# grantjr1842/delayed-streams-modeling

Measured on AMD Instinct MI355X. Metric: real-time stream throughput, stt-1b-en_fr @ bs=64 per GPU (Mimi encode + LM decode per 80 ms frame), higher is better.
Workload: dtype bf16 weights + bf16 KV, f32 activations as three exact bf16 pieces, f32 accumulate (v_mfma_f32_16x16x32_bf16); 1 GPU; stt-1b-en_fr batch=64 streaming, ring KV cache full (750 frames), Mimi encode + LM decode HIP path; streams_per_gpu=64, parallelism=replicas x1 (independent stream batches, no per-step collective), streams=encoder stream || 2 LM group stream(s)

## Files before the change

delayed-streams-modeling_amd/csrc/dsm_engine.hip:

```cpp
#include <hip/hip_runtime.h>

#include <cmath>
#include <cstdarg>
#include <cstdio>
#include <cstdlib>
#include <cstring>
#include <atomic>
#include <mutex>
#include <shared_mutex>
#include <string>
#include <set>
#include <vector>

#include "../../include/dsm.h"
#include "dsm_device.h"
#include "dsm_config_presets.h"
#include "dsm_kernels.h"
#include "dsm_numerics.h"
#include "dsm_safetensors.h"

static thread_local std::string g_create_error;

static int dsm_env_int(const char* name, int dflt) {
  const char* v = getenv(name);
// ... 163 lines not shown
};

struct LmState {
  ActScratch act;
  float *hidden = nullptr, *logits = nullptr, *eh = nullptr, *prs = nullptr;
  uint32_t *next_cb = nullptr, *text_token = nullptr, *text_out = nullptr, *codes_in = nullptr;
  uint8_t *first_step = nullptr, *mask = nullptr;
  uint32_t* rng_key = nullptr;
  unsigned long long* rng_pos = nullptr;
  uint8_t* gmask = nullptr;
  TransformerState tr;
  struct Group {
    int b0 = 0, nb = 0;
    TransformerState view;
  };
  std::vector<Group> groups;
};

struct HostItem {
  size_t step_idx = 0;
  std::vector<uint32_t> word_tokens;
  bool unended_word = false;
  double last_stop_time = 0.0;
};

}

struct dsm_engine : DsmDevice {
  dsm_asr_config cfg{};
  int B = 0;
  hipEvent_t ev_grp_in[kMaxGroups] = {}, ev_stagger[kMaxGroups] = {};
  bool grp_busy = false;
  bool serialize_groups = false;
  hipEvent_t ev_codes_consumed = nullptr;
  bool codes_consumed_valid = false;
  hipEvent_t ev_join = nullptr, ev_a = nullptr, ev_b = nullptr, ev_c = nullptr, ev_d = nullptr;
  MimiW mimi_w;
  MimiState mimi[2];
  std::atomic<bool> mimi1_ready{false};
  std::mutex mimi1_mu;
  MimiDecState dec;
  LmW lm_w;
  LmState lm;
  GraphSlot *g_enc[2] = {}, *g_grp[kMaxGroups] = {};
  float* h_pcm = nullptr;
  float* h_pcm1 = nullptr;
  uint8_t* h_mask = nullptr;
  uint32_t *h_codes = nullptr, *h_text = nullptr;
  float* h_prs = nullptr;
  std::vector<HostItem> items;
  size_t model_step_idx = 0;
  std::vector<dsm_asr_msg> msgs;
  std::vector<uint32_t> msg_tokens;
  dsm_metrics metrics{};
  static constexpr int kPipe = 4;
  struct PipeSlot {
    float* h_pcm = nullptr;
    uint8_t* h_mask = nullptr;
    uint32_t* d_codes = nullptr;
    hipEvent_t ev_done = nullptr, ev_consumed = nullptr;
    bool in_flight = false;
  };
  PipeSlot pipe[kPipe];
  int pipe_next = 0;
  bool pipe_ready = false;
  std::mutex pipe_mu;
};
// ... 520 lines not shown
template <typename WT, typename KVT, int EPI, int NT>
int launch_gemm_tiled(DsmDevice* e, hipStream_t st, GemmArgs& a) {
  int chunks = (a.Kpad + DSM_KC - 1) / DSM_KC;
  const int gx = (a.N + 63) / 64;
  const bool bx3 = e->dot_mode == 1 && sizeof(WT) == 2;
  auto ok4 = [](const RowMap& m) { return m.ld % 4 == 0 && m.bstride % 4 == 0; };
  a.vec = (a.N % 4 == 0) && (!a.Y || ok4(a.ymap)) && (!a.Y2 || ok4(a.y2map)) && (!a.res || ok4(a.rmap));
  a.chunk_loop = 0;
  if (chunks > 1 && (long)gx * ((a.M + 63) / 64) >= e->chunk_loop_min_tiles) {
    a.chunk_loop = chunks;
    a.defer_reduce = 0;
    chunks = 1;
  }
  if constexpr (EPI == EPI_GATE && NT == 2) {
    if (wk_applicable(e, sizeof(WT) == 2, a.Kpad, a.K, a.M) && chunks > 1 && a.N % 16 == 0) {
      a.ts = e->timeline ? e->dev_ts_slot(e->tag_gemm[e->sid(st)], e->sid(st), 1, 2) : nullptr;
      const int ph = e->prof_begin(e->tag_gemm[e->sid(st)], st);
      hipLaunchKernelGGL((gemm_wk_kernel<KVT, 1, 2, EPI_GATE, 1, 4, 2, true, 4>), dim3(a.N / 16, 1, (a.M + 15) / 16), dim3(256),
                         (size_t)chunks * 2 * 1024, st, a);
      e->prof_end(ph, st);
      HIPCHK(hipGetLastError());
      return 0;
    }
  }
  int MT = a.M > 32 ? 4 : (a.M > 16 ? 2 : 1);
  while (MT > 1 && (long)gx * chunks * ((a.M + 16 * MT - 1) / (16 * MT)) < 256) MT /= 2;
  if (MT == 4 && bx3 && chunks > 1 && a.M <= 64 && (long)gx * chunks <= 256 && EPI == EPI_STORE) MT = 2;
  const bool smallk = chunks == 1 && a.chunk_loop == 0 && (long)gx * ((a.M + 63) / 64) >= e->smallk_min_tiles && !bx3;
  if (smallk && e->smallk_mt < MT) MT = e->smallk_mt;
  a.ws_ntiles = (((NT - 1) * a.nt_stride) >> 4) + gx * 4;
  const int mtiles = (a.M + 15) / 16;
  if (chunks > 1) {
    const int wsid = e->sid(st);
    size_t need = (size_t)chunks * mtiles * a.ws_ntiles * 256 * sizeof(float);
    if (need > e->gemm_ws_cap[wsid]) {
      if (e->capturing) {
        e->capture_failed = true;
        e->set_error("split-K workspace grew during a graph capture");
        return DSM_ERR_STATE;
      }
      e->ws_gen += 1;
      HIPCHK(hipStreamSynchronize(st));
      if (e->gemm_ws[wsid]) HIPCHK(hipFree(e->gemm_ws[wsid]));
      e->gemm_ws[wsid] = nullptr;
      e->gemm_ws_cap[wsid] = 0;
      void* p = nullptr;
      HIPCHK(hipMalloc(&p, need));
      e->gemm_ws[wsid] = reinterpret_cast<float*>(p);
      e->gemm_ws_cap[wsid] = need;
    }
    a.ws = e->gemm_ws[wsid];
  }
  dim3 grid(gx, chunks, (a.M + 16 * MT - 1) / (16 * MT));
  const bool nt2 = NT == 1 && bx3 && a.chunk_loop > 1 && MT == 4 && (EPI == EPI_STORE || EPI == EPI_QKV) && a.N % 128 == 0 &&
                   (long)(a.N / 128) * grid.z >= 256;
  if (nt2) {
    grid.x = a.N / 128;
    a.wg_cols = 128;
    a.nt_stride = 64;
  }
  a.ts = e->timeline ? e->dev_ts_slot(e->tag_gemm[e->sid(st)], e->sid(st), 1, 2) : nullptr;
  const int ph = e->prof_begin(e->tag_gemm[e->sid(st)], st);
  const bool roll = a.chunk_loop > 1 || smallk;
  const bool deep = LoopDepth<WT, NT>::MAX == 4 && e->loop_depth == 4 && !smallk;
  if (nt2) hipLaunchKernelGGL((gemm_bx3_kernel<KVT, 4, (NT == 1 ? 2 : NT), (EPI == EPI_GATE ? EPI_STORE : EPI), true>), grid, dim3(256), 0, st, a);
  else if (MT == 4) launch_tile<WT, KVT, EPI, NT, 4>(st, grid, a, bx3, roll, deep);
  else if (MT == 2) launch_tile<WT, KVT, EPI, NT, 2>(st, grid, a, bx3, roll, deep);
  else launch_tile<WT, KVT, EPI, NT, 1>(st, grid, a, bx3, roll, deep);
  const bool rows_ok = (EPI == EPI_STORE) && a.norm_out && a.vec && !a.Y2 && a.Y && a.N <= 4096 && a.ymap.bstride == 0;
  if (chunks > 1 && !((EPI == EPI_QKV || EPI == EPI_STORE) && a.defer_reduce)) {
    if (rows_ok) {
      if (a.N <= 1024) hipLaunchKernelGGL(gemm_reduce_rows_kernel<1>, dim3(a.M), dim3(256), 0, st, a, chunks);
      else if (a.N <= 2048) hipLaunchKernelGGL(gemm_reduce_rows_kernel<2>, dim3(a.M), dim3(512), 0, st, a, chunks);
      else hipLaunchKernelGGL(gemm_reduce_rows_kernel<4>, dim3(a.M), dim3(1024), 0, st, a, chunks);
    } else {
      const int out_tiles = mtiles * ((a.N + 15) / 16);
      hipLaunchKernelGGL((gemm_reduce_kernel<KVT, EPI>), dim3((out_tiles + 3) / 4), dim3(256), 0, st, a, chunks);
    }
  }
  e->prof_end(ph, st);
  HIPCHK(hipGetLastError());
  if (a.norm_out && !(chunks > 1 && rows_ok)) {
    hipLaunchKernelGGL(row_norm_kernel, dim3(a.M), dim3(256), 0, st, a.norm_out, a.Y, a.norm_w, a.norm_b, a.M,
                       a.N, a.norm_eps, a.norm_rms);
// ... 171 lines not shown
```

delayed-streams-modeling_amd/csrc/dsm_engine_api.inc:

```

namespace {

template <typename KVT, int HD, int T>
int launch_attn_t(DsmDevice* e, hipStream_t st, float* out, const float* q, const void* k, const void* v,
                  const uint32_t* start_pos, const uint8_t* active, int B, int H, int ctx, int d, const AttnFused& fq) {
  constexpr int UNR = (sizeof(KVT) == 2 && T == 1 && HD == 128) ? 8 : 4;
  size_t lds = sizeof(float) * ((size_t)T * ctx + 4 * T * HD + 16);
  if ((long)B * H >= 2048 && (size_t)2 * ctx * HD * sizeof(KVT) >= (size_t)256 * 1024) lds += e->attn_lds_pad;
  if (lds > 64 * 1024) {
    static size_t allowed = 0;
    if (lds > allowed) {
      HIPCHK(hipFuncSetAttribute(reinterpret_cast<const void*>(&attn_kernel<KVT, HD, T, UNR>), hipFuncAttributeMaxDynamicSharedMemorySize, (int)lds));
      allowed = lds;
    }
  }
  const int tag = e->tag_attn[e->sid(st)];
  if (T == 1 && HD == 64 && ctx <= 32) {
    const int ph = e->prof_begin(tag, st);
    hipLaunchKernelGGL((attn_small_kernel<KVT, 64>), dim3((B * H + 3) / 4), dim3(256), 0, st, out, q, reinterpret_cast<const KVT*>(k),
                       reinterpret_cast<const KVT*>(v), start_pos, active, B * H, H, ctx, d, fq);
    e->prof_end(ph, st);
    HIPCHK(hipGetLastError());
    return 0;
  }
// ... 360 lines not shown
      const int per_b = T_out * (sw.out_c / 4);
      hipLaunchKernelGGL(convtr_overlap_add_kernel, dim3((per_b + 255) / 256 < 64 ? (per_b + 255) / 256 : 64, B), dim3(256), 0,
                         st, o);
      HIPCHK(hipGetLastError());
    }
    if (int rc = run_conv(e, st, sw.ra, ss.cat_ra, B, nullptr, none, ss.cat_rb, cat_map(sw.rb), nullptr, none)) return rc;
    if (i + 1 < w.dec_stages.size()) {
      if (int rc = run_conv(e, st, sw.rb, ss.cat_rb, B, nullptr, none, s.stages[i + 1].x, plain_map(B * T_out, sw.out_c), ss.y,
                            plain_map(B * T_out, sw.out_c)))
        return rc;
    } else {
      if (int rc = run_conv(e, st, sw.rb, ss.cat_rb, B, nullptr, none, s.cat_final, cat_map(w.dec_final), ss.y,
                            plain_map(B * T_out, sw.out_c)))
        return rc;
    }
  }
  if (int rc = run_conv(e, st, w.dec_final, s.cat_final, B, s.pcm, plain_map(B * DSM_FRAME_SIZE, c.channels), nullptr, none,
                        nullptr, none))
    return rc;
  if (!s.h_descs.empty()) {
    hipLaunchKernelGGL(conv_state_shift_kernel, dim3(B, (unsigned)s.h_descs.size()), dim3(256), 0, st, s.descs, s.mask,
                       s.first_call ? 1 : 0, s.started);
    HIPCHK(hipGetLastError());
  }
  s.first_call = false;
  return 0;
}

int lm_group_body(dsm_engine* e, hipStream_t st, int g, uint32_t* d_text_out, float* d_prs_out, int phase) {
  const dsm_asr_config& c = e->cfg;
  LmState& s = e->lm;
  const LmW& w = e->lm_w;
  LmState::Group& grp = s.groups[g];
  const int B = e->B, d = c.lm.d_model, b0 = grp.b0, nb = grp.nb;
  e->tag_gemm[e->sid(st)] = DSM_PROF_GEMM_LM;
  e->tag_attn[e->sid(st)] = DSM_PROF_ATTN_LM;
  uint8_t* gmask = s.gmask + b0;
  const ActScratch sc = s.act.from_row(b0, d, w.tr.hidden);
  float* hidden = s.hidden + (size_t)b0 * d;
  int rc = with_kv_type(c.kv_bf16 != 0, [&](auto kv) {
    return transformer_forward<uint16_t, decltype(kv)>(e, st, w.tr, grp.view, sc, nb, 1, gmask, nullptr, plain_map(1, 1), w.out_norm, hidden, phase);
  });
  if (rc || phase == 1) return rc;
  float* logits = s.logits + (size_t)b0 * c.text_out_vocab_size;
  {
    GemmArgs a = base_args(w.text_linear, hidden, plain_map(nb, d), nb);
    a.Y = logits; a.ymap = plain_map(nb, c.text_out_vocab_size);
    if ((rc = gemm_store<uint16_t>(e, st, a))) return rc;
  }
  if (c.temperature > 0.0f)
    hipLaunchKernelGGL(lm_gumbel_kernel, dim3(nb), dim3(256), 0, st, logits, c.text_out_vocab_size, c.temperature,
                       s.rng_key + (size_t)b0 * 8, s.rng_pos + b0, d_text_out + b0, s.text_token + b0, s.first_step + b0, gmask);
  else
    hipLaunchKernelGGL(lm_argmax_kernel, dim3(nb), dim3(256), 0, st, logits, c.text_out_vocab_size, d_text_out + b0,
                       s.text_token + b0, s.first_step + b0, gmask);
  HIPCHK(hipGetLastError());
  if (c.extra_heads_num > 0 && d_prs_out) {
    const int ehw = c.extra_heads_num * c.extra_heads_dim;
    float* eh = s.eh + (size_t)b0 * ehw;
    GemmArgs a = base_args(w.extra_heads, hidden, plain_map(nb, d), nb);
    a.Y = eh; a.ymap = plain_map(nb, ehw);
    if ((rc = gemm_store<uint16_t>(e, st, a))) return rc;
    int n = nb * c.extra_heads_num;
    hipLaunchKernelGGL(extra_heads_kernel, dim3((n + 255) / 256), dim3(256), 0, st, eh, d_prs_out + b0, nb,
                       c.extra_heads_num, c.extra_heads_dim, B);
    HIPCHK(hipGetLastError());
  }
  return 0;
}

int lm_group_head(dsm_engine* e, hipStream_t st, int g, const uint32_t* d_codes, const uint8_t* d_mask, bool with_prefix) {
  const dsm_asr_config& c = e->cfg;
  LmState& s = e->lm;
  const LmW& w = e->lm_w;
  LmState::Group& grp = s.groups[g];
  const int d = c.lm.d_model, b0 = grp.b0, nb = grp.nb, nc = c.audio_codebooks;
  uint8_t* gmask = s.gmask + b0;
  HIPCHK(hipMemcpyAsync(gmask, d_mask + b0, (size_t)nb, hipMemcpyDeviceToDevice, st));
  float* x = s.act.x + (size_t)b0 * d;
  hipLaunchKernelGGL(lm_input_kernel, dim3(nb, (d + 511) / 512), dim3(256), 0, st, x, w.text_emb, w.audio_emb,
                     d_codes + (size_t)b0 * nc, s.next_cb + (size_t)b0 * nc, s.text_token + b0, s.first_step + b0, gmask, nc, d,
                     c.audio_vocab_size, (uint32_t)c.audio_vocab_size - 1, (uint32_t)c.text_in_vocab_size - 1);
  hipLaunchKernelGGL(lm_next_codebooks_kernel, dim3((nb * nc + 255) / 256), dim3(256), 0, st, d_codes + (size_t)b0 * nc,
                     s.next_cb + (size_t)b0 * nc, gmask, nb, nc);
  HIPCHK(hipGetLastError());
  if (g > 0) HIPCHK(hipEventRecord(e->ev_grp_in[g], st));
  if (with_prefix)
    if (int rc = lm_group_body(e, st, g, nullptr, nullptr, 1)) return rc;
  return 0;
}

int lm_group_rest(dsm_engine* e, hipStream_t st, int g, uint32_t* d_text_out, float* d_prs_out, bool after_prefix) {
  const uint64_t key = (uint64_t)e->sid(st) ^ ((uint64_t)(uintptr_t)d_text_out << 3) ^ ((uint64_t)(uintptr_t)d_prs_out * 0x9E3779B97F4A7C15ull) ^
                       (after_prefix ? 0x8000000000000000ull : 0ull);
  return run_captured(e, *e->g_grp[g], st, key, [&] { return lm_group_body(e, st, g, d_text_out, d_prs_out, after_prefix ? 2 : 0); });
}

int wait_group_inputs(dsm_engine* e) {
  if (!e->grp_busy) return 0;
  for (size_t g = 1; g < e->lm.groups.size(); ++g) HIPCHK(hipStreamWaitEvent(e->s_model, e->ev_grp_in[g], 0));
  return 0;
}
int join_groups(dsm_engine* e) { return e->grp_busy ? join_groups(e, e->s_model, e->lm.groups.size()) : 0; }

int lm_step(dsm_engine* e, hipStream_t st, const uint32_t* d_codes, const uint8_t* d_mask, uint32_t* d_text_out,
            float* d_prs_out) {
  const size_t G = e->lm.groups.size();
  if (int rc = fork_groups(e, st, G)) return rc;
  const bool stagger = G > 1 && !e->serialize_groups && e->lm.groups[0].nb >= 256;
  for (size_t g = 0; g < G; ++g) {
    hipStream_t gs = (g == 0 || e->serialize_groups) ? st : e->s_grp[g];
    if (stagger && g > 0) HIPCHK(hipStreamWaitEvent(gs, e->ev_stagger[g - 1], 0));
    if (int rc = lm_group_head(e, gs, (int)g, d_codes, d_mask, stagger)) return rc;
    if (stagger && g + 1 < G) HIPCHK(hipEventRecord(e->ev_stagger[g], gs));
  }
  if (int rc = run_groups(e, st, G, e->serialize_groups,
                          [&](size_t g, hipStream_t gs) { return lm_group_rest(e, gs, (int)g, d_text_out, d_prs_out, stagger); }))
    return rc;
  if (G > 1) e->grp_busy = true;
// ... 177 lines not shown
  if (c.extra_heads_num > 0) {
    std::vector<float> eh((size_t)c.extra_heads_num * c.extra_heads_dim * d);
    for (int i = 0; i < c.extra_heads_num && !ld.failed; ++i) {
      auto w = ld.get((int64_t)c.extra_heads_dim * d, "extra_heads.%d.weight", i);
      memcpy(&eh[(size_t)i * c.extra_heads_dim * d], w.data(), sizeof(float) * w.size());
    }
    if (ld.failed) return DSM_ERR_IO;
    if (int rc = pack_linear(e, &e->lm_w.extra_heads, eh.data(), c.extra_heads_num * c.extra_heads_dim, d, true, nullptr)) return rc;
  }
  return 0;
}

static int create_impl(dsm_engine* e, const dsm_asr_config* cfg, int device_id, int batch_size, const char* lm_path,
                       const char* mimi_path, const void* attach_arena = nullptr, size_t attach_bytes = 0,
                       const uint8_t* attach_manifest = nullptr, size_t attach_manifest_bytes = 0) {
  e->cfg = *cfg;
  e->B = batch_size;
  const dsm_asr_config& c = e->cfg;
  if (batch_size <= 0) { e->set_error("batch_size must be positive"); return DSM_ERR_INVALID; }
  if (c.audio_codebooks > 64 || c.audio_codebooks != c.mimi.quantizer_n_q) {
    e->set_error("audio_codebooks (%d) must equal the Mimi quantizer_n_q (%d) and be <= 64", c.audio_codebooks,
                 c.mimi.quantizer_n_q);
    return DSM_ERR_INVALID;
  }
  if (c.mimi.n_residual_layers != 1) {
    e->set_error("only n_residual_layers = 1 (dilation 1 residual blocks, Mimi v0_1) is supported");
    return DSM_ERR_INVALID;
  }
  if (c.extra_heads_num > DSM_MAX_EXTRA_HEADS) { e->set_error("too many extra heads"); return DSM_ERR_INVALID; }
  if (c.dot_mode != 0 && c.dot_mode != 1) { e->set_error("dot_mode must be 0 (f32 MFMA chain) or 1 (bx3)"); return DSM_ERR_INVALID; }
  for (const dsm_transformer_config* t : {&c.lm, &c.mimi.transformer})
    if (int rc = check_transformer_config(e, *t)) return rc;
  if (int rc = e->open(device_id, c.dot_mode, true)) return rc;
  for (hipEvent_t* ev : {&e->ev_join, &e->ev_codes_consumed})
    if (int rc = e->new_event(ev)) return rc;
  for (hipEvent_t* ev : {&e->ev_a, &e->ev_b, &e->ev_c, &e->ev_d})
    if (int rc = e->new_event(ev, hipEventDefault)) return rc;
  for (auto& gs : e->g_enc) gs = e->graph_slot();
  const int B = batch_size, d = c.lm.d_model;
  if (attach_arena) {
    e->arena = const_cast<char*>(reinterpret_cast<const char*>(attach_arena));
    e->arena_size = attach_bytes;
    e->arena_owned = false;
    e->manifest.assign(attach_manifest, attach_manifest + attach_manifest_bytes);
    e->manifest_pos = 0;
    e->arena_off = 0;
    e->wmode = dsm_engine::W_ATTACH;
    if (int rc = load_all_weights(e, nullptr, nullptr)) return rc;
    if (e->arena_off != e->arena_size || e->manifest_pos != e->manifest.size()) {
      e->set_error("received weight arena does not match this configuration (%zu of %zu bytes, %zu of %zu manifest entries used)",
                   e->arena_off, e->arena_size, e->manifest_pos, e->manifest.size());
      return DSM_ERR_INVALID;
    }
  } else {
    char err[512];
    dsm_st_file* fm = dsm_st_open(mimi_path, err, sizeof err);
    if (!fm) { e->set_error("%s", err); return DSM_ERR_IO; }
    dsm_st_file* fl = dsm_st_open(lm_path, err, sizeof err);
    if (!fl) { dsm_st_close(fm); e->set_error("%s", err); return DSM_ERR_IO; }
    e->wmode = dsm_engine::W_MEASURE;
    e->arena_off = 0;
    int rc = load_all_weights(e, fl, fm);
    if (rc == 0) {
      e->arena_size = e->arena_off;
      void* p = nullptr;
      hipError_t he = hipMalloc(&p, e->arena_size);
      if (he != hipSuccess) { e->set_error("hipMalloc of the %zu-byte weight arena failed: %s", e->arena_size, hipGetErrorString(he)); rc = DSM_ERR_DEVICE; }
      else {
// ... 27 lines not shown
  if (int rc = e->dalloc(&s.next_cb, (size_t)B * c.audio_codebooks)) return rc;
  if (int rc = e->dalloc(&s.text_token, B)) return rc;
  if (int rc = e->dalloc(&s.text_out, B)) return rc;
  if (int rc = e->dalloc(&s.codes_in, (size_t)B * c.audio_codebooks)) return rc;
  if (int rc = e->dalloc(&s.first_step, B)) return rc;
  if (int rc = e->dalloc(&s.rng_key, (size_t)B * 8)) return rc;
  if (int rc = e->dalloc(&s.rng_pos, B)) return rc;
  {
    std::vector<uint32_t> keys((size_t)B * 8);
    for (int b = 0; b < B; ++b) dsm_seed_from_u64(0x5EED0000ull + (uint64_t)b, &keys[(size_t)b * 8]);
    HIPCHK(hipMemcpy(s.rng_key, keys.data(), sizeof(uint32_t) * keys.size(), hipMemcpyHostToDevice));
    HIPCHK(hipStreamSynchronize(nullptr));
  }
  if (int rc = e->dalloc(&s.mask, B)) return rc;
  if (int rc = alloc_transformer_state(e, &s.tr, c.lm, B, 1, c.kv_bf16 != 0)) return rc;
  if (int rc = e->dalloc(&s.gmask, B)) return rc;
  {
    int G = dsm_env_int("DSM_LM_GROUPS", B >= 32 ? 2 : 1);
    if (G < 1) G = 1;
    if (G > dsm_engine::kMaxGroups) G = dsm_engine::kMaxGroups;
    const int n16 = (B + 15) / 16;
    if (G > n16) G = n16;
    s.groups.resize(G);
    int b0 = 0;
    for (int g = 0; g < G; ++g) {
      int blocks = n16 / G + (g < n16 % G ? 1 : 0);
      int nb = std::min(blocks * 16, B - b0);
      LmState::Group& grp = s.groups[g];
      grp.b0 = b0;
      grp.nb = nb;
      grp.view = group_view(s.tr, c.lm, c.kv_bf16 ? 2 : 4, b0);
      b0 += nb;
      e->g_grp[g] = e->graph_slot();
      if (g > 0)
        if (int rc = e->new_event(&e->ev_grp_in[g])) return rc;
    }
    if (int rc = e->open_groups(G)) return rc;
    for (int g = 0; g + 1 < G; ++g)
      if (int rc = e->new_event(&e->ev_stagger[g])) return rc;
  }
  {
    long n = (long)B * c.audio_codebooks;
    hipLaunchKernelGGL(fill_u32_kernel, dim3((unsigned)((n + 255) / 256)), dim3(256), 0, e->s_model, s.next_cb,
                       (uint32_t)c.audio_vocab_size - 1, n);
    hipLaunchKernelGGL(fill_u32_kernel, dim3((unsigned)((B + 255) / 256)), dim3(256), 0, e->s_model, s.text_token,
                       (uint32_t)c.text_in_vocab_size - 1, (long)B);
    HIPCHK(hipGetLastError());
    HIPCHK(hipMemsetAsync(s.first_step, 1, B, e->s_model));
  }
  e->items.assign(B, HostItem());
  if (int rc = e->halloc(&e->h_pcm, (size_t)B * DSM_FRAME_SIZE)) return rc;
  if (int rc = e->halloc(&e->h_pcm1, (size_t)B * DSM_FRAME_SIZE)) return rc;
  if (int rc = e->halloc(&e->h_mask, (size_t)B)) return rc;
  if (int rc = e->halloc(&e->h_codes, (size_t)B * c.audio_codebooks)) return rc;
  if (int rc = e->halloc(&e->h_text, (size_t)B)) return rc;
  if (int rc = e->halloc(&e->h_prs, (size_t)B * (c.extra_heads_num + 1))) return rc;
  HIPCHK(hipDeviceSynchronize());
  e->metrics.algorithmic_bytes_lm = lm_algorithmic_bytes(e);
  e->metrics.algorithmic_bytes_encode = mimi_enc_algorithmic_bytes(e);
  return 0;
}

int dsm_asr_create(const dsm_asr_config* cfg, int device_id, int batch_size, const char* lm_safetensors,
                   const char* mimi_safetensors, dsm_engine** out) {
  if (!cfg || !out || !lm_safetensors || !mimi_safetensors) {
    g_create_error = "null argument";
    return DSM_ERR_INVALID;
  }
// ... 341 lines not shown
  HIPCHK(hipSetDevice(e->device));
  ApiShared api(e);
  if (int rc = dsm_sync(e)) return rc;
  uint32_t key[8];
  dsm_seed_from_u64(seed, key);
  const unsigned long long zero = 0;
  HIPCHK(hipMemcpy(e->lm.rng_key + (size_t)slot * 8, key, sizeof key, hipMemcpyHostToDevice));
  HIPCHK(hipMemcpy(e->lm.rng_pos + slot, &zero, sizeof zero, hipMemcpyHostToDevice));
  return dsm_sync(e);
}

int dsm_mimi_reset_slot(dsm_engine* e, int slot) {
  if (!e) return DSM_ERR_INVALID;
  if (slot < 0 || slot >= e->B) {
    e->set_error("batch index out of range: %d >= %d", slot, e->B);
    return DSM_ERR_INVALID;
  }
  HIPCHK(hipSetDevice(e->device));
  ApiShared api(e);
  return reset_mimi_slot(e, 0, e->s_enc, slot);
}

int dsm_get_metrics(dsm_engine* e, dsm_metrics* out) {
  if (!e || !out) return DSM_ERR_INVALID;
  *out = e->metrics;
  e->fill_graph_metrics(out);
  return 0;
}

int dsm_mimi_encode_step_dev(dsm_engine* e, const float* d_pcm, const uint8_t* d_mask, uint32_t* d_codes_out) {
  if (!e || !d_pcm || !d_mask) return DSM_ERR_INVALID;
  HIPCHK(hipSetDevice(e->device));
  ApiShared api(e);
  if (e->codes_consumed_valid) HIPCHK(hipStreamWaitEvent(e->s_enc, e->ev_codes_consumed, 0));
  if (int rc = upload_pcm(e, 0, e->s_enc, d_pcm, hipMemcpyDeviceToDevice)) return rc;
  HIPCHK(hipMemcpyAsync(e->mimi[0].mask, d_mask, (size_t)e->B, hipMemcpyDeviceToDevice, e->s_enc));
  if (int rc = mimi_encode(e, 0, e->s_enc)) return rc;
  if (d_codes_out)
    HIPCHK(hipMemcpyAsync(d_codes_out, e->mimi[0].codes, sizeof(uint32_t) * (size_t)e->B * e->cfg.mimi.quantizer_n_q,
                          hipMemcpyDeviceToDevice, e->s_enc));
  HIPCHK(hipEventRecord(e->ev_join, e->s_enc));
  e->metrics.steps_encode += 1;
  return 0;
}

int dsm_asr_step_tokens_dev(dsm_engine* e, const uint32_t* d_codes, const uint8_t* d_mask, uint32_t* d_text_tokens_out,
                            float* d_vad_prs_out) {
  if (!e || !d_mask) return DSM_ERR_INVALID;
  HIPCHK(hipSetDevice(e->device));
  ApiShared api(e);
  if (int rc = wait_group_inputs(e)) return rc;
  HIPCHK(hipMemcpyAsync(e->lm.mask, d_mask, (size_t)e->B, hipMemcpyDeviceToDevice, e->s_model));
  const uint32_t* codes = d_codes;
  if (!codes) {
    HIPCHK(hipStreamWaitEvent(e->s_model, e->ev_join, 0));
    HIPCHK(hipMemcpyAsync(e->lm.codes_in, e->mimi[0].codes, sizeof(uint32_t) * (size_t)e->B * e->cfg.audio_codebooks,
                          hipMemcpyDeviceToDevice, e->s_model));
    HIPCHK(hipEventRecord(e->ev_codes_consumed, e->s_model));
    e->codes_consumed_valid = true;
    codes = e->lm.codes_in;
  }
  if (int rc = lm_step(e, e->s_model, codes, e->lm.mask, d_text_tokens_out ? d_text_tokens_out : e->lm.text_out,
                       e->cfg.extra_heads_num > 0 ? (d_vad_prs_out ? d_vad_prs_out : e->lm.prs) : nullptr))
    return rc;
  e->metrics.steps_lm += 1;
  e->model_step_idx += 1;
  return 0;
}

int dsm_asr_step_pcm_dev(dsm_engine* e, const float* d_pcm, const uint8_t* d_mask, uint32_t* d_codes_out,
                         uint32_t* d_text_tokens_out, float* d_vad_prs_out) {
  if (!e || !d_pcm || !d_mask) return DSM_ERR_INVALID;
  HIPCHK(hipSetDevice(e->device));
  if (int rc = ensure_model_side_mimi(e)) return rc;
  ApiShared api(e);
  hipStream_t st = e->s_model;
  if (int rc = wait_group_inputs(e)) return rc;
  if (int rc = upload_pcm(e, 1, st, d_pcm, hipMemcpyDeviceToDevice)) return rc;
  HIPCHK(hipMemcpyAsync(e->mimi[1].mask, d_mask, (size_t)e->B, hipMemcpyDeviceToDevice, st));
  if (int rc = mimi_encode(e, 1, st)) return rc;
  if (d_codes_out)
    HIPCHK(hipMemcpyAsync(d_codes_out, e->mimi[1].codes, sizeof(uint32_t) * (size_t)e->B * e->cfg.mimi.quantizer_n_q,
                          hipMemcpyDeviceToDevice, st));
  if (int rc = lm_step(e, st, e->mimi[1].codes, e->mimi[1].mask, d_text_tokens_out ? d_text_tokens_out : e->lm.text_out,
                       e->cfg.extra_heads_num > 0 ? (d_vad_prs_out ? d_vad_prs_out : e->lm.prs) : nullptr))
    return rc;
  e->metrics.steps_encode += 1;
  e->metrics.steps_lm += 1;
  e->model_step_idx += 1;
  return 0;
}

int dsm_prof_enable(dsm_engine* e, unsigned tag_mask) {
  if (!e) return DSM_ERR_INVALID;
  e->prof_mask = tag_mask;
// ... 171 lines not shown
```

delayed-streams-modeling_amd/csrc/dsm_kernels.h:

```cpp
#pragma once
#include <hip/hip_runtime.h>
#include <stdint.h>
#include "dsm_numerics.h"
#include "dsm_sampling.h"

typedef float f32x4 __attribute__((ext_vector_type(4)));
typedef short dsm_bf16x8 __attribute__((ext_vector_type(8)));

__device__ __forceinline__ float wave_sum64(float v) {
#pragma unroll
  for (int off = 32; off >= 1; off >>= 1) v = v + __shfl_xor(v, off, 64);
  return v;
}

enum { EPI_STORE = 0, EPI_QKV = 1, EPI_GATE = 2, EPI_RVQ = 3 };

struct RowMap {
  long bstride;
  int rpb;
  int ld;
  int toff;
  __host__ __device__ long off(int m) const { return (long)(m / rpb) * bstride + (long)((m % rpb) + toff) * ld; }
};

struct GemmArgs {
  const float* X;
  RowMap xmap;
  const void* W;
  int Kpad, K, N, M;
  int nt_stride;
  int wpacked;
  int w_ntiles;
  int wg_cols;
  const float* bias;
  const float* scale;
  const float* res;
  RowMap rmap;
  float* Y;
  RowMap ymap;
  float* Y2;
  RowMap y2map;
  int act;
  int vec;
  int d, hd, H, T, ctx;
  void* kcache;
  void* vcache;
  const uint32_t* widx;
  const float* rope_cs;
  const uint8_t* active;
  float* pval;
  uint32_t* pidx;
  float* ws;
  int ws_ntiles;
  int defer_reduce;
  int chunk_loop;
  const float* norm_w;
  const float* norm_b;
  float* norm_out;
  float norm_eps;
  int norm_rms;
  unsigned long long* ts;
};

template <typename WT>
__device__ __forceinline__ const WT* dsm_wbase(const GemmArgs& a, const WT* W, int n0, int r, int q) {
  if (sizeof(WT) == 2 && a.wpacked) return W + ((long)(n0 >> 4) * (a.Kpad >> 5)) * 512 + (q * 16 + r) * 8;
  return W + (long)(n0 + r) * a.Kpad + 8 * q;
}
template <typename WT>
__device__ __forceinline__ int dsm_wstep(const GemmArgs& a) { return (sizeof(WT) == 2 && a.wpacked) ? 16 : 1; }

__device__ __forceinline__ void launch_stamp_begin(unsigned long long* ts) {
  if (!ts || threadIdx.x != 0) return;
  const unsigned lin = blockIdx.x + gridDim.x * (blockIdx.y + gridDim.y * blockIdx.z);
  if (lin < 128) atomicMin(&ts[0], wall_clock64());
}
__device__ __forceinline__ void launch_stamp_end(unsigned long long* ts) {
  if (!ts || threadIdx.x != 0) return;
  const unsigned total = gridDim.x * gridDim.y * gridDim.z;
  const unsigned lin = blockIdx.x + gridDim.x * (blockIdx.y + gridDim.y * blockIdx.z);
  if (lin + 512 >= total) atomicMax(&ts[1], wall_clock64());
}

template <typename WT>
__device__ __forceinline__ void load_w8(const WT* p, float (&o)[8]);
template <>
__device__ __forceinline__ void load_w8<uint16_t>(const uint16_t* p, float (&o)[8]) {
// ... 1214 lines not shown
                                  const uint8_t* __restrict__ active, uint32_t* __restrict__ start_pos,
                                  uint32_t* __restrict__ widx, float* __restrict__ rope_cs,
                                  const float* __restrict__ inv_freq, int B, int T, int ctx, int hd,
                                  int rope_before) {
  const int b = blockIdx.x;
  if (b >= B) return;
  __shared__ uint32_t s_pos_after;
  if (threadIdx.x == 0) {
    uint32_t p = pos[b], i = idx[b];
    const uint32_t p0 = p;
    start_pos[b] = p;
    for (int t = 0; t < T; ++t) widx[b * T + t] = active[b] ? (uint32_t)((i + t) % ctx) : i;
    if (active[b]) {
      pos[b] = p + T;
      idx[b] = (uint32_t)((i + T) % ctx);
      p += T;
    }
    s_pos_after = rope_before ? p0 : p;
  }
  __syncthreads();
  if (rope_cs) {
    const int half = hd / 2;
    for (int e = threadIdx.x; e < T * half; e += blockDim.x) {
      int t = e / half, i = e % half;
      float ang = (float)(s_pos_after + (uint32_t)t) * inv_freq[i];
      float s, c;
      dsm_sincosf(ang, &s, &c);
      rope_cs[((long)(b * T + t) * half + i) * 2] = c;
      rope_cs[((long)(b * T + t) * half + i) * 2 + 1] = s;
    }
  }
}

__global__ void lm_input_kernel(float* __restrict__ x, const uint16_t* __restrict__ text_emb,
                                const uint16_t* __restrict__ audio_emb ,
                                const uint32_t* __restrict__ codes , uint32_t* __restrict__ next_cb,
                                const uint32_t* __restrict__ text_token, const uint8_t* __restrict__ first_step,
                                const uint8_t* __restrict__ active, int nc, int d, int audio_vocab,
                                uint32_t pad_tok, uint32_t start_tok) {
  const int b = blockIdx.x;
  __shared__ uint32_t toks[64];
  const bool first = first_step[b] != 0;
  if (threadIdx.x < nc) toks[threadIdx.x] = first ? pad_tok : next_cb[b * nc + threadIdx.x];
  __syncthreads();
  const uint32_t tt = first ? start_tok : text_token[b];
  const int j = (blockIdx.y * blockDim.x + threadIdx.x) * 2;
  if (j < d) {
    uint32_t t2 = *reinterpret_cast<const uint32_t*>(text_emb + (long)tt * d + j);
    float e0 = __uint_as_float(t2 << 16), e1 = __uint_as_float(t2 & 0xFFFF0000u);
    for (int i = 0; i < nc; ++i) {
      uint32_t a2 = *reinterpret_cast<const uint32_t*>(audio_emb + ((long)i * audio_vocab + toks[i]) * d + j);
      e0 = e0 + __uint_as_float(a2 << 16);
      e1 = e1 + __uint_as_float(a2 & 0xFFFF0000u);
    }
    *reinterpret_cast<float2*>(x + (long)b * d + j) = make_float2(e0, e1);
  }
}

__global__ void lm_next_codebooks_kernel(const uint32_t* __restrict__ codes, uint32_t* __restrict__ next_cb,
                                         const uint8_t* __restrict__ active, int B, int nc) {
  const int i = blockIdx.x * blockDim.x + threadIdx.x;
  if (i < B * nc && active[i / nc]) next_cb[i] = codes[i];
}

__device__ inline int block_argmax_first(const float* __restrict__ lg, int V) {
  float bv = -DSM_INF_F;
  int bi = 0x7FFFFFFF;
  for (int j = threadIdx.x; j < V; j += blockDim.x) {
    float v = lg[j];
    if (v > bv || (v == bv && j < bi)) { bv = v; bi = j; }
  }
  __shared__ float sv[256];
  __shared__ int si[256];
  sv[threadIdx.x] = bv;
  si[threadIdx.x] = bi;
  __syncthreads();
  for (int off = blockDim.x / 2; off >= 1; off >>= 1) {
    if ((int)threadIdx.x < off) {
      float ov = sv[threadIdx.x + off];
      int oi = si[threadIdx.x + off];
      if (ov > sv[threadIdx.x] || (ov == sv[threadIdx.x] && oi < si[threadIdx.x])) {
        sv[threadIdx.x] = ov;
        si[threadIdx.x] = oi;
      }
    }
    __syncthreads();
  }
  const int r = si[0] == 0x7FFFFFFF ? 0 : si[0];
  __syncthreads();
  return r;
}

__global__ void lm_argmax_kernel(const float* __restrict__ logits, int V, uint32_t* __restrict__ text_out,
                                 uint32_t* __restrict__ text_token, uint8_t* __restrict__ first_step,
                                 const uint8_t* __restrict__ active) {
  const int b = blockIdx.x;
  const uint32_t tok = (uint32_t)block_argmax_first(logits + (long)b * V, V);
// ... 315 lines not shown
  else
    tok = (uint32_t)block_argmax_first(logits, V);
  if (threadIdx.x == 0) {
    lat[(long)b * S + k] = tok;
    const uint32_t nt = (forced[b] && k > 0) ? pad : tok;
    last_tok[b] = nt;
    s_next = nt;
  }
  if (!next.x) return;
  }
  __syncthreads();
  const uint32_t t = s_next;
  for (int j = 0; j < next.rps; ++j) {
    if (j > 0) __syncthreads();
    dep_head_row(next, b * next.rps + j, t, hred);
  }
}

__global__ void extra_heads_kernel(const float* __restrict__ eh , float* __restrict__ prs, int B,
                                   int nh, int dim, int prs_stride ) {
  int i = blockIdx.x * blockDim.x + threadIdx.x;
  if (i >= B * nh) return;
  int b = i / nh, h = i % nh;
  const float* lg = eh + ((long)b * nh + h) * dim;
  float m = lg[0];
  for (int k = 1; k < dim; ++k) m = lg[k] > m ? lg[k] : m;
  float sum = 0.0f, e0 = 0.0f;
  for (int k = 0; k < dim; ++k) {
    float e = dsm_expf(lg[k] - m);
    if (k == 0) e0 = e;
    sum = sum + e;
  }
  prs[(long)h * prs_stride + b] = e0 / sum;
}

struct SeanetFrontArgs {
  const float* cat_init;
  const float *w0, *b0;
  const float *w1, *b1;
  const float *w2, *b2;
  float* cat_ra;
  float* cat_down;
  int ld0, ld1, ld2;
  int T, S0, Sd;
};

template <int TM>
constexpr size_t seanet_front_lds() { return sizeof(float) * ((TM + 2) * 64 + TM * 64 + TM * 32 + (TM + 2 + 7 - 1)); }
template <int TM>
__global__ __launch_bounds__(256) void seanet_front_kernel(SeanetFrontArgs a) {
  constexpr int C0 = 64, C1 = 32, TAPS0 = 7, MTILES = TM / 16;
  static_assert(TM == 64 || TM == 32, "tile");
  extern __shared__ __attribute__((aligned(16))) float front_lds[];
  float* e0 = front_lds;
  float* y0 = e0 + (TM + 2) * C0;
  float* hs = y0 + TM * C0;
  float* xs = hs + TM * C1;
  const int tid = threadIdx.x, lane = tid & 63, wave = tid >> 6;
  const int r = lane & 15, q = lane >> 4;
  const int b = blockIdx.y, t0 = blockIdx.x * TM;
  const bool first = t0 == 0, last = t0 + TM == a.T;
  const float* cat = a.cat_init + (long)b * (a.S0 + a.T);
  for (int i = tid; i < TM + 2 + TAPS0 - 1; i += 256) {
    const int c = t0 - 2 + i;
    xs[i] = c >= 0 ? cat[c] : 0.0f;
  }
// ... 449 lines not shown
```

Measured before the change: 1822 x realtime (stream-seconds of audio per wall second).

## Fuse LM step head and tail into single kernels and drop codes copy

Replaces the LM input embedding, next-codebook copy, mask copy, position/ring-index update, RoPE sin/cos and first-layer norm with one per-row lm_head_kernel. For greedy decoding it also defers the split-K reduction of the text and extra-heads GEMMs into a single lm_tail_kernel that reduces, argmaxes and computes VAD probabilities. The encoder's codes are read in place, and the encoder now waits on each group's input event instead of a separate copy event. This cuts kernel launches and small memcpys per step, at the cost of more intricate cross-stream ordering and workspace offset handling.

```diff
diff --git a/delayed-streams-modeling_amd/csrc/dsm_engine.hip b/delayed-streams-modeling_amd/csrc/dsm_engine.hip
--- a/delayed-streams-modeling_amd/csrc/dsm_engine.hip
+++ b/delayed-streams-modeling_amd/csrc/dsm_engine.hip
@@ -219,7 +219,6 @@
   hipEvent_t ev_grp_in[kMaxGroups] = {}, ev_stagger[kMaxGroups] = {};
   bool grp_busy = false;
   bool serialize_groups = false;
-  hipEvent_t ev_codes_consumed = nullptr;
   bool codes_consumed_valid = false;
   hipEvent_t ev_join = nullptr, ev_a = nullptr, ev_b = nullptr, ev_c = nullptr, ev_d = nullptr;
   MimiW mimi_w;
@@ -806,7 +805,7 @@
   const int mtiles = (a.M + 15) / 16;
   if (chunks > 1) {
     const int wsid = e->sid(st);
-    size_t need = (size_t)chunks * mtiles * a.ws_ntiles * 256 * sizeof(float);
+    size_t need = ((size_t)a.ws_off + (size_t)chunks * mtiles * a.ws_ntiles * 256) * sizeof(float);
     if (need > e->gemm_ws_cap[wsid]) {
       if (e->capturing) {
         e->capture_failed = true;
@@ -823,7 +822,7 @@
       e->gemm_ws[wsid] = reinterpret_cast<float*>(p);
       e->gemm_ws_cap[wsid] = need;
     }
-    a.ws = e->gemm_ws[wsid];
+    a.ws = e->gemm_ws[wsid] + a.ws_off;
   }
   dim3 grid(gx, chunks, (a.M + 16 * MT - 1) / (16 * MT));
   const bool nt2 = NT == 1 && bx3 && a.chunk_loop > 1 && MT == 4 && (EPI == EPI_STORE || EPI == EPI_QKV) && a.N % 128 == 0 &&
diff --git a/delayed-streams-modeling_amd/csrc/dsm_engine_api.inc b/delayed-streams-modeling_amd/csrc/dsm_engine_api.inc
--- a/delayed-streams-modeling_amd/csrc/dsm_engine_api.inc
+++ b/delayed-streams-modeling_amd/csrc/dsm_engine_api.inc
@@ -416,40 +416,84 @@
   LmState& s = e->lm;
   const LmW& w = e->lm_w;
   LmState::Group& grp = s.groups[g];
-  const int B = e->B, d = c.lm.d_model, b0 = grp.b0, nb = grp.nb;
+  const int B = e->B, d = c.lm.d_model, b0 = grp.b0, nb = grp.nb, V = c.text_out_vocab_size;
   e->tag_gemm[e->sid(st)] = DSM_PROF_GEMM_LM;
   e->tag_attn[e->sid(st)] = DSM_PROF_ATTN_LM;
   uint8_t* gmask = s.gmask + b0;
   const ActScratch sc = s.act.from_row(b0, d, w.tr.hidden);
   float* hidden = s.hidden + (size_t)b0 * d;
   int rc = with_kv_type(c.kv_bf16 != 0, [&](auto kv) {
-    return transformer_forward<uint16_t, decltype(kv)>(e, st, w.tr, grp.view, sc, nb, 1, gmask, nullptr, plain_map(1, 1), w.out_norm, hidden, phase);
+    return transformer_forward<uint16_t, decltype(kv)>(e, st, w.tr, grp.view, sc, nb, 1, gmask, nullptr, plain_map(1, 1), w.out_norm, hidden,
+                                                       phase, nullptr, true);
   });
   if (rc || phase == 1) return rc;
-  float* logits = s.logits + (size_t)b0 * c.text_out_vocab_size;
-  {
-    GemmArgs a = base_args(w.text_linear, hidden, plain_map(nb, d), nb);
-    a.Y = logits; a.ymap = plain_map(nb, c.text_out_vocab_size);
-    if ((rc = gemm_store<uint16_t>(e, st, a))) return rc;
-  }
-  if (c.temperature > 0.0f)
-    hipLaunchKernelGGL(lm_gumbel_kernel, dim3(nb), dim3(256), 0, st, logits, c.text_out_vocab_size, c.temperature,
-                       s.rng_key + (size_t)b0 * 8, s.rng_pos + b0, d_text_out + b0, s.text_token + b0, s.first_step + b0, gmask);
-  else
-    hipLaunchKernelGGL(lm_argmax_kernel, dim3(nb), dim3(256), 0, st, logits, c.text_out_vocab_size, d_text_out + b0,
-                       s.text_token + b0, s.first_step + b0, gmask);
+  float* logits = s.logits + (size_t)b0 * V;
+  const bool heads = c.extra_heads_num > 0 && d_prs_out;
+  const int ehw = c.extra_heads_num * c.extra_heads_dim;
+  float* eh = s.eh + (size_t)b0 * ehw;
+  auto deferrable = [](const Linear& L) { return L.Kpad > DSM_KC && L.K % 32 == 0 && !L.bias; };
+  const bool fused = c.temperature <= 0.0f && V % 4 == 0 && V + ehw <= 12 * 1024  &&
+                     deferrable(w.text_linear) && (!heads || deferrable(w.extra_heads));
+  if (!fused) {
+    {
+      GemmArgs a = base_args(w.text_linear, hidden, plain_map(nb, d), nb);
+      a.Y = logits; a.ymap = plain_map(nb, V);
+      if ((rc = gemm_store<uint16_t>(e, st, a))) return rc;
+    }
+    if (c.temperature > 0.0f)
+      hipLaunchKernelGGL(lm_gumbel_kernel, dim3(nb), dim3(256), 0, st, logits, V, c.temperature, s.rng_key + (size_t)b0 * 8,
+                         s.rng_pos + b0, d_text_out + b0, s.text_token + b0, s.first_step + b0, gmask);
+    else
+      hipLaunchKernelGGL(lm_argmax_kernel, dim3(nb), dim3(256), 0, st, logits, V, d_text_out + b0, s.text_token + b0,
+                         s.first_step + b0, gmask);
+    HIPCHK(hipGetLastError());
+    if (heads) {
+      GemmArgs a = base_args(w.extra_heads, hidden, plain_map(nb, d), nb);
+      a.Y = eh; a.ymap = plain_map(nb, ehw);
+      if ((rc = gemm_store<uint16_t>(e, st, a))) return rc;
+      int n = nb * c.extra_heads_num;
+      hipLaunchKernelGGL(extra_heads_kernel, dim3((n + 255) / 256), dim3(256), 0, st, eh, d_prs_out + b0, nb,
+                         c.extra_heads_num, c.extra_heads_dim, B);
+      HIPCHK(hipGetLastError());
+    }
+    return 0;
+  }
+  LmTailArgs t;
+  memset(&t, 0, sizeof t);
+  auto deferred = [&](const Linear& L, float* Y, int N, long ws_off, LogitSrc& src, long& ws_floats) {
+    GemmArgs a = base_args(L, hidden, plain_map(nb, d), nb);
+    a.Y = Y; a.ymap = plain_map(nb, N);
+    a.defer_reduce = 1;
+    a.ws_off = ws_off;
+    if (int r = gemm_store<uint16_t>(e, st, a)) return r;
+    src = LogitSrc{};
+    src.rps = 1;
+    ws_floats = 0;
+    if (a.defer_reduce) {
+      src.ws = a.ws;
+      src.ld = (long)a.ws_ntiles * 16;
+      src.cstride = (long)((nb + 15) / 16) * 16 * src.ld;
+      src.chunks = (a.Kpad + DSM_KC - 1) / DSM_KC;
+      src.store = Y;
+      ws_floats = src.cstride * src.chunks;
+    } else {
+      src.rows = Y;
+    }
+    return 0;
+  };
+  long text_floats = 0, eh_floats = 0;
+  if ((rc = deferred(w.text_linear, logits, V, 0, t.text, text_floats))) return rc;
+  if (heads) {
+    const uint64_t gen = e->ws_gen;
+    if ((rc = deferred(w.extra_heads, eh, ehw, text_floats, t.eh, eh_floats))) return rc;
+    if (e->ws_gen != gen && (rc = deferred(w.text_linear, logits, V, 0, t.text, text_floats))) return rc;
+    t.nh = c.extra_heads_num; t.dim = c.extra_heads_dim;
+    t.prs = d_prs_out + b0; t.prs_stride = B;
+  }
+  t.V = V;
+  t.text_out = d_text_out + b0; t.text_token = s.text_token + b0; t.first_step = s.first_step + b0; t.active = gmask;
+  hipLaunchKernelGGL(lm_tail_kernel, dim3(nb), dim3(256), sizeof(float) * (size_t)(V + t.nh * t.dim), st, t);
   HIPCHK(hipGetLastError());
-  if (c.extra_heads_num > 0 && d_prs_out) {
-    const int ehw = c.extra_heads_num * c.extra_heads_dim;
-    float* eh = s.eh + (size_t)b0 * ehw;
-    GemmArgs a = base_args(w.extra_heads, hidden, plain_map(nb, d), nb);
-    a.Y = eh; a.ymap = plain_map(nb, ehw);
-    if ((rc = gemm_store<uint16_t>(e, st, a))) return rc;
-    int n = nb * c.extra_heads_num;
-    hipLaunchKernelGGL(extra_heads_kernel, dim3((n + 255) / 256), dim3(256), 0, st, eh, d_prs_out + b0, nb,
-                       c.extra_heads_num, c.extra_heads_dim, B);
-    HIPCHK(hipGetLastError());
-  }
   return 0;
 }
 
@@ -458,17 +502,25 @@
   LmState& s = e->lm;
   const LmW& w = e->lm_w;
   LmState::Group& grp = s.groups[g];
-  const int d = c.lm.d_model, b0 = grp.b0, nb = grp.nb, nc = c.audio_codebooks;
-  uint8_t* gmask = s.gmask + b0;
-  HIPCHK(hipMemcpyAsync(gmask, d_mask + b0, (size_t)nb, hipMemcpyDeviceToDevice, st));
-  float* x = s.act.x + (size_t)b0 * d;
-  hipLaunchKernelGGL(lm_input_kernel, dim3(nb, (d + 511) / 512), dim3(256), 0, st, x, w.text_emb, w.audio_emb,
-                     d_codes + (size_t)b0 * nc, s.next_cb + (size_t)b0 * nc, s.text_token + b0, s.first_step + b0, gmask, nc, d,
-                     c.audio_vocab_size, (uint32_t)c.audio_vocab_size - 1, (uint32_t)c.text_in_vocab_size - 1);
-  hipLaunchKernelGGL(lm_next_codebooks_kernel, dim3((nb * nc + 255) / 256), dim3(256), 0, st, d_codes + (size_t)b0 * nc,
-                     s.next_cb + (size_t)b0 * nc, gmask, nb, nc);
+  const dsm_transformer_config& tc = w.tr.cfg;
+  const int d = tc.d_model, b0 = grp.b0, nb = grp.nb, nc = c.audio_codebooks;
+  LmHeadArgs h;
+  memset(&h, 0, sizeof h);
+  h.x = s.act.x + (size_t)b0 * d; h.xn = s.act.xn + (size_t)b0 * d;
+  h.text_emb = w.text_emb; h.audio_emb = w.audio_emb;
+  h.codes = d_codes + (size_t)b0 * nc; h.next_cb = s.next_cb + (size_t)b0 * nc;
+  h.text_token = s.text_token + b0; h.first_step = s.first_step + b0;
+  h.mask = d_mask + b0; h.gmask = s.gmask + b0;
+  h.nc = nc; h.d = d; h.audio_vocab = c.audio_vocab_size;
+  h.pad_tok = (uint32_t)c.audio_vocab_size - 1; h.start_tok = (uint32_t)c.text_in_vocab_size - 1;
+  h.pos = grp.view.pos; h.idx = grp.view.idx; h.start_pos = grp.view.start_pos; h.widx = grp.view.widx;
+  h.rope_cs = tc.positional_embedding == 1 ? grp.view.rope_cs : nullptr;
+  h.inv_freq = w.tr.inv_freq;
+  h.ctx = tc.context; h.hd = d / tc.num_heads; h.rope_before = w.tr.rope_pos_before ? 1 : 0;
+  h.nw = w.tr.layers[0].n1w; h.nb = w.tr.layers[0].n1b; h.eps = norm_eps(tc.norm); h.rms = tc.norm;
+  hipLaunchKernelGGL(lm_head_kernel, dim3(nb), dim3(256), 0, st, h);
   HIPCHK(hipGetLastError());
-  if (g > 0) HIPCHK(hipEventRecord(e->ev_grp_in[g], st));
+  HIPCHK(hipEventRecord(e->ev_grp_in[g], st));
   if (with_prefix)
     if (int rc = lm_group_body(e, st, g, nullptr, nullptr, 1)) return rc;
   return 0;
@@ -712,8 +764,7 @@
   for (const dsm_transformer_config* t : {&c.lm, &c.mimi.transformer})
     if (int rc = check_transformer_config(e, *t)) return rc;
   if (int rc = e->open(device_id, c.dot_mode, true)) return rc;
-  for (hipEvent_t* ev : {&e->ev_join, &e->ev_codes_consumed})
-    if (int rc = e->new_event(ev)) return rc;
+  if (int rc = e->new_event(&e->ev_join)) return rc;
   for (hipEvent_t* ev : {&e->ev_a, &e->ev_b, &e->ev_c, &e->ev_d})
     if (int rc = e->new_event(ev, hipEventDefault)) return rc;
   for (auto& gs : e->g_enc) gs = e->graph_slot();
@@ -807,8 +858,7 @@
       grp.view = group_view(s.tr, c.lm, c.kv_bf16 ? 2 : 4, b0);
       b0 += nb;
       e->g_grp[g] = e->graph_slot();
-      if (g > 0)
-        if (int rc = e->new_event(&e->ev_grp_in[g])) return rc;
+      if (int rc = e->new_event(&e->ev_grp_in[g])) return rc;
     }
     if (int rc = e->open_groups(G)) return rc;
     for (int g = 0; g + 1 < G; ++g)
@@ -1216,7 +1266,8 @@
   if (!e || !d_pcm || !d_mask) return DSM_ERR_INVALID;
   HIPCHK(hipSetDevice(e->device));
   ApiShared api(e);
-  if (e->codes_consumed_valid) HIPCHK(hipStreamWaitEvent(e->s_enc, e->ev_codes_consumed, 0));
+  if (e->codes_consumed_valid)
+    for (size_t g = 0; g < e->lm.groups.size(); ++g) HIPCHK(hipStreamWaitEvent(e->s_enc, e->ev_grp_in[g], 0));
   if (int rc = upload_pcm(e, 0, e->s_enc, d_pcm, hipMemcpyDeviceToDevice)) return rc;
   HIPCHK(hipMemcpyAsync(e->mimi[0].mask, d_mask, (size_t)e->B, hipMemcpyDeviceToDevice, e->s_enc));
   if (int rc = mimi_encode(e, 0, e->s_enc)) return rc;
@@ -1233,18 +1284,13 @@
   if (!e || !d_mask) return DSM_ERR_INVALID;
   HIPCHK(hipSetDevice(e->device));
   ApiShared api(e);
-  if (int rc = wait_group_inputs(e)) return rc;
-  HIPCHK(hipMemcpyAsync(e->lm.mask, d_mask, (size_t)e->B, hipMemcpyDeviceToDevice, e->s_model));
   const uint32_t* codes = d_codes;
   if (!codes) {
     HIPCHK(hipStreamWaitEvent(e->s_model, e->ev_join, 0));
-    HIPCHK(hipMemcpyAsync(e->lm.codes_in, e->mimi[0].codes, sizeof(uint32_t) * (size_t)e->B * e->cfg.audio_codebooks,
-                          hipMemcpyDeviceToDevice, e->s_model));
-    HIPCHK(hipEventRecord(e->ev_codes_consumed, e->s_model));
+    codes = e->mimi[0].codes;
     e->codes_consumed_valid = true;
-    codes = e->lm.codes_in;
-  }
-  if (int rc = lm_step(e, e->s_model, codes, e->lm.mask, d_text_tokens_out ? d_text_tokens_out : e->lm.text_out,
+  }
+  if (int rc = lm_step(e, e->s_model, codes, d_mask, d_text_tokens_out ? d_text_tokens_out : e->lm.text_out,
                        e->cfg.extra_heads_num > 0 ? (d_vad_prs_out ? d_vad_prs_out : e->lm.prs) : nullptr))
     return rc;
   e->metrics.steps_lm += 1;
diff --git a/delayed-streams-modeling_amd/csrc/dsm_kernels.h b/delayed-streams-modeling_amd/csrc/dsm_kernels.h
--- a/delayed-streams-modeling_amd/csrc/dsm_kernels.h
+++ b/delayed-streams-modeling_amd/csrc/dsm_kernels.h
@@ -53,6 +53,7 @@
   float* ws;
   int ws_ntiles;
   int defer_reduce;
+  long ws_off;
   int chunk_loop;
   const float* norm_w;
   const float* norm_b;
@@ -1333,37 +1334,6 @@
   }
 }
 
-__global__ void lm_input_kernel(float* __restrict__ x, const uint16_t* __restrict__ text_emb,
-                                const uint16_t* __restrict__ audio_emb ,
-                                const uint32_t* __restrict__ codes , uint32_t* __restrict__ next_cb,
-                                const uint32_t* __restrict__ text_token, const uint8_t* __restrict__ first_step,
-                                const uint8_t* __restrict__ active, int nc, int d, int audio_vocab,
-                                uint32_t pad_tok, uint32_t start_tok) {
-  const int b = blockIdx.x;
-  __shared__ uint32_t toks[64];
-  const bool first = first_step[b] != 0;
-  if (threadIdx.x < nc) toks[threadIdx.x] = first ? pad_tok : next_cb[b * nc + threadIdx.x];
-  __syncthreads();
-  const uint32_t tt = first ? start_tok : text_token[b];
-  const int j = (blockIdx.y * blockDim.x + threadIdx.x) * 2;
-  if (j < d) {
-    uint32_t t2 = *reinterpret_cast<const uint32_t*>(text_emb + (long)tt * d + j);
-    float e0 = __uint_as_float(t2 << 16), e1 = __uint_as_float(t2 & 0xFFFF0000u);
-    for (int i = 0; i < nc; ++i) {
-      uint32_t a2 = *reinterpret_cast<const uint32_t*>(audio_emb + ((long)i * audio_vocab + toks[i]) * d + j);
-      e0 = e0 + __uint_as_float(a2 << 16);
-      e1 = e1 + __uint_as_float(a2 & 0xFFFF0000u);
-    }
-    *reinterpret_cast<float2*>(x + (long)b * d + j) = make_float2(e0, e1);
-  }
-}
-
-__global__ void lm_next_codebooks_kernel(const uint32_t* __restrict__ codes, uint32_t* __restrict__ next_cb,
-                                         const uint8_t* __restrict__ active, int B, int nc) {
-  const int i = blockIdx.x * blockDim.x + threadIdx.x;
-  if (i < B * nc && active[i / nc]) next_cb[i] = codes[i];
-}
-
 __device__ inline int block_argmax_first(const float* __restrict__ lg, int V) {
   float bv = -DSM_INF_F;
   int bi = 0x7FFFFFFF;
@@ -1745,6 +1715,157 @@
     sum = sum + e;
   }
   prs[(long)h * prs_stride + b] = e0 / sum;
+}
+
+struct LmHeadArgs {
+  float* x;
+  float* xn;
+  const uint16_t* text_emb;
+  const uint16_t* audio_emb;
+  const uint32_t* codes;
+  uint32_t* next_cb;
+  const uint32_t* text_token;
+  const uint8_t* first_step;
+  const uint8_t* mask;
+  uint8_t* gmask;
+  int nc, d, audio_vocab;
+  uint32_t pad_tok, start_tok;
+  uint32_t *pos, *idx, *start_pos, *widx;
+  float* rope_cs;
+  const float* inv_freq;
+  int ctx, hd, rope_before;
+  const float* nw;
+  const float* nb;
+  float eps;
+  int rms;
+};
+__global__ __launch_bounds__(256) void lm_head_kernel(LmHeadArgs h) {
+  __shared__ uint32_t toks[64];
+  __shared__ float red[8];
+  __shared__ uint32_t s_pos_after;
+  const int b = blockIdx.x, d = h.d, nc = h.nc;
+  const uint8_t mk = h.mask[b];
+  const bool first = h.first_step[b] != 0;
+  if ((int)threadIdx.x < nc) toks[threadIdx.x] = first ? h.pad_tok : h.next_cb[b * nc + threadIdx.x];
+  if (threadIdx.x == 0) {
+    h.gmask[b] = mk;
+    uint32_t p = h.pos[b];
+    const uint32_t i = h.idx[b], p0 = p;
+    h.start_pos[b] = p;
+    h.widx[b] = mk ? (uint32_t)(i % h.ctx) : i;
+    if (mk) {
+      h.pos[b] = p + 1;
+      h.idx[b] = (uint32_t)((i + 1) % h.ctx);
+      p += 1;
+    }
+    s_pos_after = h.rope_before ? p0 : p;
+  }
+  __syncthreads();
+  if ((int)threadIdx.x < nc && mk) h.next_cb[b * nc + threadIdx.x] = h.codes[b * nc + threadIdx.x];
+  if (h.rope_cs) {
+    const int half = h.hd / 2;
+    for (int i = threadIdx.x; i < half; i += blockDim.x) {
+      const float ang = (float)s_pos_after * h.inv_freq[i];
+      float s, c;
+      dsm_sincosf(ang, &s, &c);
+      h.rope_cs[((long)b * half + i) * 2] = c;
+      h.rope_cs[((long)b * half + i) * 2 + 1] = s;
+    }
+  }
+  const uint32_t tt = first ? h.start_tok : h.text_token[b];
+  float4 v[DSM_ROW_ITS];
+  float s = 0.0f, s2 = 0.0f;
+#pragma unroll
+  for (int it = 0; it < DSM_ROW_ITS; ++it) {
+    const int i = it * 1024 + 4 * (int)threadIdx.x;
+    v[it] = make_float4(0.f, 0.f, 0.f, 0.f);
+    if (i < d) {
+      const uint2 t2 = *reinterpret_cast<const uint2*>(h.text_emb + (long)tt * d + i);
+      float e0 = __uint_as_float(t2.x << 16), e1 = __uint_as_float(t2.x & 0xFFFF0000u);
+      float e2 = __uint_as_float(t2.y << 16), e3 = __uint_as_float(t2.y & 0xFFFF0000u);
+      for (int c0 = 0; c0 < nc; c0 += 8) {
+        uint2 a2[8];
+#pragma unroll
+        for (int u = 0; u < 8; ++u) {
+          const int c = c0 + u < nc ? c0 + u : nc - 1;
+          a2[u] = *reinterpret_cast<const uint2*>(h.audio_emb + ((long)c * h.audio_vocab + toks[c]) * d + i);
+        }
+#pragma unroll
+        for (int u = 0; u < 8; ++u)
+          if (c0 + u < nc) {
+            e0 = e0 + __uint_as_float(a2[u].x << 16);
+            e1 = e1 + __uint_as_float(a2[u].x & 0xFFFF0000u);
+            e2 = e2 + __uint_as_float(a2[u].y << 16);
+            e3 = e3 + __uint_as_float(a2[u].y & 0xFFFF0000u);
+          }
+      }
+      v[it] = make_float4(e0, e1, e2, e3);
+      *reinterpret_cast<float4*>(h.x + (long)b * d + i) = v[it];
+      s = s + v[it].x; s2 = DSM_FMAF(v[it].x, v[it].x, s2);
+      s = s + v[it].y; s2 = DSM_FMAF(v[it].y, v[it].y, s2);
+      s = s + v[it].z; s2 = DSM_FMAF(v[it].z, v[it].z, s2);
+      s = s + v[it].w; s2 = DSM_FMAF(v[it].w, v[it].w, s2);
+    }
+  }
+  block_row_sums(s, s2, red);
+  row_norm_apply(v, s, s2, d, h.eps, h.rms, h.nw, h.nb, h.xn + (long)b * d);
+}
+
+struct LmTailArgs {
+  LogitSrc text;
+  int V;
+  uint32_t* text_out;
+  uint32_t* text_token;
+  uint8_t* first_step;
+  const uint8_t* active;
+  LogitSrc eh;
+  int nh, dim;
+  float* prs;
+  int prs_stride;
+};
+__global__ __launch_bounds__(256) void lm_tail_kernel(LmTailArgs a) {
+  extern __shared__ __attribute__((aligned(16))) unsigned char smem[];
+  float* logits = reinterpret_cast<float*>(smem);
+  float* ehs = logits + a.V;
+  const int b = blockIdx.x, V = a.V, ehw = a.nh * a.dim;
+  for (int i = threadIdx.x; i < ehw; i += blockDim.x) {
+    float t;
+    if (a.eh.ws) {
+      const float* p = a.eh.ws + (long)b * a.eh.ld + i;
+      t = p[0];
+      for (int c = 1; c < a.eh.chunks; ++c) t = t + p[c * a.eh.cstride];
+      a.eh.store[(long)b * ehw + i] = t;
+    } else {
+      t = a.eh.rows[(long)b * ehw + i];
+    }
+    ehs[i] = t;
+  }
+  for (int j = 4 * (int)threadIdx.x; j < V; j += 4 * (int)blockDim.x) {
+    const f32x4 o = logit4(a.text, b, V, j);
+    if (a.text.ws) *reinterpret_cast<f32x4*>(a.text.store + (long)b * V + j) = o;
+    *reinterpret_cast<f32x4*>(logits + j) = o;
+  }
+  __syncthreads();
+  const uint32_t tok = (uint32_t)block_argmax_first(logits, V);
+  if (threadIdx.x == 0) {
+    a.text_out[b] = tok;
+    if (a.active[b]) {
+      a.text_token[b] = tok;
+      a.first_step[b] = 0;
+    }
+  }
+  if ((int)threadIdx.x < a.nh) {
+    const float* lg = ehs + threadIdx.x * a.dim;
+    float m = lg[0];
+    for (int k = 1; k < a.dim; ++k) m = lg[k] > m ? lg[k] : m;
+    float sum = 0.0f, e0 = 0.0f;
+    for (int k = 0; k < a.dim; ++k) {
+      const float e = dsm_expf(lg[k] - m);
+      if (k == 0) e0 = e;
+      sum = sum + e;
+    }
+    a.prs[(long)threadIdx.x * a.prs_stride + b] = e0 / sum;
+  }
 }
 
 struct SeanetFrontArgs {
```

Result: no change. 1817 x realtime (stream-seconds of audio per wall second) (-0.3%).
